# liuhatry/xflow

Measured on AMD Instinct MI355X. Metric: samples/sec (whole node) + logloss, LR-FTRL Criteo-1TB shape at 1/2/4/8 MI355X, higher is better.
Workload: dtype fp32; 1 GPU; model=LR-FTRL, global_batch=262144, seq_len=39, parallelism=dp1+table-shard1, rows_per_gpu=262144, nnz_per_row=39, slices=1, grad_layout=unique_lr, hashed_features=1000000000, table_slots_per_gpu=2147483648, backend=hip:gfx950:0, a2a_transport=none, input_overlap=False, table_growths=0

## Files before the change

### csrc/engine/engine.cpp

```cpp
#include <cstdlib>
#include "xflow/engine.h"

#include <algorithm>
#include <atomic>
#include <chrono>
#include <cmath>
#include <cstdio>
#include <cstring>
#include <thread>
#include <fstream>
#include <stdexcept>

namespace xflow {

namespace {

uint64_t next_pow2(uint64_t v) {
  uint64_t p = 1;
  while (p < v) p <<= 1;
  return p;
}

constexpr char kMagic[8] = {'X', 'F', 'L', 'O', 'W', 'T', 'B', '1'};

// ... 43 lines not shown
  table_.split = 0;
  table_.cap = 1ull << log2_cap_;
  const u64 seg = 1ull << table_.seg_log2;
  table_.probe_limit = seg < kMaxProbe ? seg : kMaxProbe;
  max_segs_ = cfg_.table_grow ? (1ull << max_log2_cap_) >> table_.seg_log2 : table_.cap >> table_.seg_log2;
  table_bytes_ = (size_t)table_.cap * table_.L.stride * sizeof(u32);
  table_.words = static_cast<u32*>(
      be.table_reserve((size_t)(max_segs_ << table_.seg_log2) * table_.L.stride * sizeof(u32),
                       max_segs_ > (table_.cap >> table_.seg_log2)));
  table_range_.e = this;
  table_.words = static_cast<u32*>(be.table_commit(table_.words, table_bytes_));
  overflow_ = mon_.alloc_zero(be, 4) + 2;
  table_.size = reinterpret_cast<unsigned long long*>(mon_.get());
  table_.overflow = overflow_ + 1;
  be.table_clear(table_);
  if (cfg_.admit_min_count > 1) {
    const int top = cfg_.table_grow ? max_log2_cap_ : log2_cap_;
    admit_.log2 = cfg_.admit_log2 ? cfg_.admit_log2 : (top + 1 < kAdmitMaxLog2 ? top + 1 : kAdmitMaxLog2);
    if (admit_.log2 < kAdmitBlockLog2) admit_.log2 = kAdmitBlockLog2;
    admit_.min_count = cfg_.admit_min_count;
    admit_.counters = admit_counters_.alloc_zero(be, (size_t)1 << admit_.log2);
  }
  std::memset(snaps_.alloc(be, kSnaps), 0, sizeof(HostSnap) * kSnaps);

  const int64_t nnz = cfg_.max_nnz;
  scratch_.cap = next_pow2((uint64_t)((double)nnz * cfg_.scratch_factor) + 1);
  scratch_.keys = scratch_keys_.alloc(be, scratch_.cap);
  be.fill_u64(scratch_.keys, kEmptyKey, scratch_.cap);
  scratch_.stamps = scratch_stamps_.alloc_zero(be, scratch_.cap);
  scratch_.claims = scratch_claims_.alloc_zero(be, 1);
  scratch_.rebuild_at = scratch_.cap / 2;
  scratch_.epoch = 0;
  if (be.is_gpu()) {
    scratch_.ctl = scratch_ctl_.alloc(be, 5);
    unsigned long long c0[5] = {scratch_.cap, 0ull, 0ull, 0ull, 0ull};
    be.copy_h2d(scratch_.ctl, c0, sizeof(c0));
  }
  block_counts_.alloc(be, scratch_.cap / 4096 + 1);

  const int ps = cfg_.model.pstride();
  uniq_keys_.alloc(be, nnz);
  uniq_slot_.alloc(be, nnz);
  use_worker_set(0);
  const uint64_t rows1 = scratch_.cap + 1;
  grad_.alloc_zero(be, rows1 * slice_cap_ * ps);
  tmask_.alloc_zero(be, rows1);
  const bool fm_ref = cfg_.model.kind == kFM && cfg_.model.fm_math == kFmReference;
  const bool fm_std = cfg_.model.kind == kFM && cfg_.model.fm_math == kFmStandard;
  const bool mvm = cfg_.model.kind == kMVM && cfg_.model.kernel_dim() >= 2;
  if (be.is_gpu() && (cfg_.model.kind == kLR || fm_ref || fm_std || mvm)) {
    const bool vec = fm_std || mvm;
    const int kd = cfg_.model.kernel_dim();
    const int nv = fm_ref ? 2 : (fm_std ? 1 + kd : (mvm ? kd : 1));
    const int shift = red_shift(nv);
    const int recw = vec ? vec_rec_words(nv) / 2 : nv;
    const int group_rows = fm_ref ? kFmGroupRows : (vec ? kFmStdMinGroupRows : kLrGroupRows);
    const uint64_t dests = scratch_.cap * (uint64_t)slice_cap_;
    const int vd = nv - 1;
    const int maxb = vec && (cfg_.max_rows + fmstd_block(vd) - 1) / fmstd_block(vd) <= kSegMaxGroups
                         ? vec_red_max_buckets(vd)
                         : kRedMaxBuckets;
    red_maxb_ = vec ? maxb : 0;
    int nb = (int)((dests + (1ull << shift) - 1) >> shift);
    int nsub = 1;
    while ((uint64_t)nb > (uint64_t)maxb * nsub) nsub <<= 1;
    if (nsub > 1) nb = maxb;
    red_nsub_ = nsub;
    if (nb <= maxb && dests < (1ull << 32)) {
      const int64_t groups = (cfg_.max_rows + group_rows - 1) / group_rows;
// ... 1205 lines not shown
    be_->copy_d2h(&c0, admit_.counters + p.c0, 1);
    be_->copy_d2h(&c1, admit_.counters + p.c1, 1);
    out[i] = c0 < c1 ? c0 : c1;
  }
  return out;
}

void Engine::admit_export(uint8_t* dst) {
  if (admit_.counters) be_->copy_d2h(dst, admit_.counters, admit_bytes());
}

void Engine::admit_import(const uint8_t* src) {
  if (!admit_.counters) throw std::runtime_error("admit_import: admission is off");
  be_->synchronize();
  be_->copy_h2d(admit_.counters, src, admit_bytes());
  be_->synchronize();
}

std::vector<u32> Engine::server_slots(int buf) {
  if (buf < 0 || buf >= kSrvBufs) throw std::invalid_argument("server buffer must be in [0, kSrvBufs)");
  const SrvBuf& sb = srv_[buf];
  std::vector<u32> out((size_t)(sb.n > 0 ? sb.n : 0));
  if (!out.empty()) be_->copy_d2h(out.data(), sb.slots, sizeof(u32) * out.size());
  return out;
}

int64_t Engine::scratch_capacity() {
  if (!scratch_.ctl) return (int64_t)scratch_.cap;
  unsigned long long c = 0;
  be_->copy_d2h(&c, scratch_.ctl, sizeof(c));
  return (int64_t)c;
}

bool Engine::overflowed() {
  u32 o[2] = {0, 0};
  be_->copy_d2h(o, overflow_, sizeof(o));
  return o[0] || o[1];
}

BatchView Engine::synth_batch(const SynthArgs& a0, int64_t slice_rows) {
  SynthArgs a = a0;
  if (a.rows > cfg_.max_rows || a.rows * a.fields > cfg_.max_nnz)
    throw std::invalid_argument("synth batch exceeds engine capacity");
  if (a.col_stride > 0 && (a.col_stride < a.rows || (!a0.keys && a.col_stride != a.rows)))
    throw std::invalid_argument("synth: col_stride must be >= rows (== rows for staging)");
  a.keys = a0.keys ? a0.keys : st_keys_;
  a.labels = a0.labels ? a0.labels : st_labels_;
  if (!a0.fgid) a.fgid = cfg_.model.kind == kMVM ? st_fgid_.get() : nullptr;
  be_->synth_batch(a);
  BatchView b;
  b.keys = a.keys;
  b.labels = a.labels;
  b.fgid = a.fgid;
  b.rows = a.rows;
  b.nnz = a.rows * a.fields;
  b.nnz_per_row = a.fields;
  b.slice_rows = slice_rows;
  b.col_stride = a.col_stride;
  return b;
}

BatchView Engine::stage_host_batch(const BatchView& h) {
  if (h.rows > cfg_.max_rows || h.nnz > cfg_.max_nnz)
    throw std::invalid_argument("host batch exceeds engine capacity");
  BatchView b = h;
  be_->copy_h2d(st_keys_, h.keys, sizeof(u64) * h.nnz);
// ... 228 lines not shown
```

### csrc/hip/kernels_table.hip

```cpp
#include <cstdlib>
#include <cstring>
#include <type_traits>

#include "kernels.h"
#include "hip_util.h"

namespace xflow {
namespace hip {

constexpr u32 kNoSlot = 0xFFFFFFFFu;
constexpr int kGroupGridCap = 8192;

__device__ __forceinline__ u64 active_cap(const ScratchView& sv) {
  return sv.ctl ? (u64)sv.ctl[0] : sv.cap;
}

__device__ __forceinline__ u64 batch_cap(const ScratchView& sv) {
  return sv.ctl ? (u64)sv.ctl[3] : sv.cap;
}

__device__ __forceinline__ bool batch_spilled(const ScratchView& sv) {
  return sv.ctl && sv.ctl[4] == (unsigned long long)sv.epoch;
}

// ... 158 lines not shown
    else pos[i] = (u32)e;
  }
  block_count_add<kBlock>(sv.claims, claimed);
}

constexpr int kCompactItems = 16;
constexpr int kCompactChunk = kBlock * kCompactItems;
constexpr int kScanBlock = 1024;

__device__ __forceinline__ unsigned int compact_hits(const ScratchView& sv, u64 base, u64 cap,
                                                     unsigned int& cnt) {
  unsigned int hit = 0;
  cnt = 0;
  if (base >= cap) return 0;
  const uint4 q = *reinterpret_cast<const uint4*>(sv.stamps + base);
  const u32 w[4] = {q.x, q.y, q.z, q.w};
  const u32 e = sv.epoch & 0xFFu;
#pragma unroll
  for (int j = 0; j < 16; ++j) hit |= (unsigned int)(((w[j >> 2] >> (8 * (j & 3))) & 0xFFu) == e) << j;
  cnt = __popc(hit);
  return hit;
}

__global__ void __launch_bounds__(kBlock) k_compact_count(ScratchView sv,
                                                          unsigned int* __restrict__ counts) {
  const u64 base = (u64)blockIdx.x * kCompactChunk + (u64)threadIdx.x * kCompactItems;
  unsigned int cnt;
  compact_hits(sv, base, batch_spilled(sv) ? sv.cap : active_cap(sv), cnt);
  unsigned int tot;
  block_exclusive_scan<kBlock>(cnt, &tot);
  if (threadIdx.x == 0) counts[blockIdx.x] = tot;
}

__global__ void __launch_bounds__(kScanBlock) k_compact_scan(
    unsigned int* __restrict__ counts, int nb, unsigned long long* __restrict__ n_out,
    unsigned long long* __restrict__ claims, unsigned long long* __restrict__ ctl,
    u64 cap_alloc, unsigned long long* __restrict__ n_copy,
    unsigned long long* __restrict__ cap_out, u32 epoch) {
  if (ctl) {
    const u64 lim = ctl[4] == epoch ? cap_alloc : (u64)ctl[0];
    const u64 nbl = (lim + kCompactChunk - 1) / kCompactChunk;
    if (nbl < (u64)nb) nb = (int)nbl;
  }
  unsigned long long carry = 0;
  for (int c0 = 0; c0 < nb; c0 += kScanBlock) {
    int i = c0 + (int)threadIdx.x;
    unsigned int v = i < nb ? counts[i] : 0u;
    unsigned int tot;
    unsigned int ex = block_exclusive_scan<kScanBlock>(v, &tot);
    if (i < nb) counts[i] = (unsigned int)(carry + ex);
    carry += tot;
  }
  if (threadIdx.x == 0) {
    *n_out = carry;
    if (n_copy) *n_copy = carry;
    if (ctl) {
      const u64 mx = ctl[1] > carry ? ctl[1] : carry;
      ctl[1] = mx;
      u64 want = kScratchMinCap;
      while (want < kScratchHeadroom * mx && want < cap_alloc) want <<= 1;
      if (want > cap_alloc) want = cap_alloc;
      const u64 cur = ctl[0];
      const bool rebuild = *claims > cur / 2 || want > cur || want * 4 <= cur;
      ctl[3] = cur;
      ctl[2] = rebuild ? want : 0ull;
      if (rebuild) {
        ctl[0] = want;
        *claims = 0ull;
      }
    }
    if (cap_out) *cap_out = ctl && ctl[4] != epoch ? ctl[3] : cap_alloc;
  }
}

__global__ void __launch_bounds__(kBlock) k_compact_write(ScratchView sv,
                                                          const unsigned int* __restrict__ offs,
                                                          u64* __restrict__ uk,
                                                          u32* __restrict__ up,
                                                          u32* __restrict__ inv) {
  const u64 base = (u64)blockIdx.x * kCompactChunk + (u64)threadIdx.x * kCompactItems;
  unsigned int cnt;
  unsigned int hit = compact_hits(sv, base, batch_spilled(sv) ? sv.cap : batch_cap(sv), cnt);
  unsigned int tot;
  unsigned int ex = block_exclusive_scan<kBlock>(cnt, &tot);
  unsigned long long dst = (unsigned long long)offs[blockIdx.x] + ex;
  u32 iv[kCompactItems];
  u64 kv[kCompactItems];
  if (hit) {
    const ulonglong2* kp = reinterpret_cast<const ulonglong2*>(sv.keys + base);
#pragma unroll
    for (int q = 0; q < kCompactItems / 2; ++q) {
      const ulonglong2 v = kp[q];
      kv[2 * q] = v.x;
      kv[2 * q + 1] = v.y;
    }
  }
#pragma unroll
  for (int j = 0; j < kCompactItems; ++j) {
    iv[j] = 0xFFFFFFFFu;
    if (!(hit & (1u << j))) continue;
    u64 s = base + (u64)j;
    uk[dst] = kv[j];
    up[dst] = (u32)s;
    iv[j] = (u32)dst;
    ++dst;
  }
  if (inv && hit) {
    uint4* ip = reinterpret_cast<uint4*>(inv + base);
#pragma unroll
    for (int j = 0; j < kCompactItems / 4; ++j)
      ip[j] = make_uint4(iv[4 * j], iv[4 * j + 1], iv[4 * j + 2], iv[4 * j + 3]);
  }
  const u64 fresh = sv.ctl ? (u64)sv.ctl[2] : 0ull;
  if (base < fresh) {
    ulonglong2* kp = reinterpret_cast<ulonglong2*>(sv.keys + base);
#pragma unroll
    for (int j = 0; j < kCompactItems / 2; ++j) kp[j] = make_ulonglong2(kEmptyKey, kEmptyKey);
  }
}

constexpr int kRemapPer = 4;

__global__ void __launch_bounds__(kBlock) k_remap_pos(u32* __restrict__ pos, int64_t nnz,
                                                      const u32* __restrict__ inv, u32 none) {
  const int64_t i = ((int64_t)blockIdx.x * kBlock + threadIdx.x) * kRemapPer;
  auto map = [&](u32 u) { return u == 0xFFFFFFFFu ? none : u; };
  if (i + kRemapPer <= nnz) {
    uint4 p[kRemapPer / 4];
#pragma unroll
    for (int q = 0; q < kRemapPer / 4; ++q) p[q] = reinterpret_cast<const uint4*>(pos + i)[q];
    u32 u[kRemapPer];
#pragma unroll
    for (int q = 0; q < kRemapPer / 4; ++q) {
      u[4 * q] = inv[p[q].x];
      u[4 * q + 1] = inv[p[q].y];
      u[4 * q + 2] = inv[p[q].z];
      u[4 * q + 3] = inv[p[q].w];
    }
#pragma unroll
    for (int q = 0; q < kRemapPer / 4; ++q)
      reinterpret_cast<uint4*>(pos + i)[q] =
          make_uint4(map(u[4 * q]), map(u[4 * q + 1]), map(u[4 * q + 2]), map(u[4 * q + 3]));
  } else {
    for (int64_t j = i; j < nnz; ++j) pos[j] = map(inv[pos[j]]);
  }
}

void launch_remap_pos(u32* pos, int64_t nnz, const u32* inv, u32 none, hipStream_t st) {
  if (nnz <= 0) return;
  if (reinterpret_cast<uintptr_t>(pos) & 15) throw std::runtime_error("remap_pos: pos must be 16-byte aligned");
// ... 35 lines not shown

void launch_partition_counts(const ScratchView& s, const u32* chunk_offsets,
                             const int64_t* n_uniq, int64_t* counts, int64_t seq, hipStream_t st) {
  if (s.parts < 2 || s.parts > kMaxParts) throw std::runtime_error("partition_counts: bad parts");
  hipLaunchKernelGGL(k_partition_counts, dim3(1), dim3(kPartBlock), 0, st, s, chunk_offsets,
                     n_uniq, counts, seq);
  XF_HIP_CHECK(hipGetLastError());
}

void launch_dedup(const u64* keys, int64_t nnz, ScratchView s, DedupOut o, hipStream_t st) {
  if (nnz <= 0) return;
  if (!s.ctl || s.grow > 0.0f) {
    if (s.ctl) hipLaunchKernelGGL(k_scratch_grow, dim3(1), dim3(1), 0, st, s.ctl, s.cap, s.grow);
    hipLaunchKernelGGL(k_scratch_maybe_clear, dim3(grid_for((int64_t)s.cap)), dim3(kBlock), 0, st,
                       s.keys, s.cap, s.claims, s.rebuild_at, s.ctl);
    hipLaunchKernelGGL(k_scratch_claims_reset, dim3(1), dim3(1), 0, st, s.claims, s.rebuild_at,
                       s.ctl);
  }
  int g1 = (int)((nnz + kDedupChunk - 1) / kDedupChunk);
  if (o.lead) {
    if (nnz % kDedupChunk || s.cap >= kLeadBit || s.parts != 1)
      throw std::runtime_error("dedup: the leader handoff needs whole tiles and < 2^31 slots");
    hipLaunchKernelGGL(k_dedup_insert<true>, dim3(g1), dim3(kBlock), 0, st, keys, nnz, s, o.pos,
                       o.overflow);
  } else {
    hipLaunchKernelGGL(k_dedup_insert<false>, dim3(g1), dim3(kBlock), 0, st, keys, nnz, s, o.pos,
                       o.overflow);
  }
  if (!o.block_counts) throw std::runtime_error("dedup: block_counts workspace missing");
  int g2 = (int)((s.cap + kCompactChunk - 1) / kCompactChunk);
  hipLaunchKernelGGL(k_compact_count, dim3(g2), dim3(kBlock), 0, st, s, o.block_counts);
  hipLaunchKernelGGL(k_compact_scan, dim3(1), dim3(kScanBlock), 0, st, o.block_counts, g2,
                     reinterpret_cast<unsigned long long*>(o.n_uniq), s.claims, s.ctl, s.cap,
                     reinterpret_cast<unsigned long long*>(o.n_uniq_copy), o.cap_out, s.epoch);
  hipLaunchKernelGGL(k_compact_write, dim3(g2), dim3(kBlock), 0, st, s, o.block_counts,
                     o.uniq_keys, o.uniq_pos, o.inv);
  XF_HIP_CHECK(hipGetLastError());
}

__global__ void k_fill_u64(u64* p, u64 v, size_t n) {
  const size_t stride = (size_t)gridDim.x * blockDim.x;
  for (size_t i = (size_t)blockIdx.x * blockDim.x + threadIdx.x; i < n; i += stride) p[i] = v;
}

struct SmallBytes {
  unsigned char b[256];
};

__global__ void k_upload_small(unsigned char* __restrict__ dst, SmallBytes v, int n) {
  for (int i = threadIdx.x; i < n; i += blockDim.x) dst[i] = v.b[i];
}

void launch_upload_small(void* dst, const void* src, size_t bytes, hipStream_t st) {
  if (bytes == 0) return;
  if (bytes > sizeof(SmallBytes)) throw std::runtime_error("upload_small: at most 256 bytes");
  SmallBytes v;
  std::memcpy(v.b, src, bytes);
  hipLaunchKernelGGL(k_upload_small, dim3(1), dim3(64), 0, st, static_cast<unsigned char*>(dst),
                     v, (int)bytes);
  XF_HIP_CHECK(hipGetLastError());
}

__global__ void k_download_small(unsigned char* __restrict__ dst,
                                 const unsigned char* __restrict__ src, int n) {
  for (int i = threadIdx.x; i < n; i += blockDim.x) dst[i] = src[i];
}

// ... 1740 lines not shown
```

### csrc/include/xflow/backend.h

```cpp
#pragma once

#include <stddef.h>
#include <stdint.h>

#include <memory>
#include <stdexcept>
#include <string>
#include <vector>

#include "xflow/types.h"

namespace xflow {

constexpr u64 kMaxProbe = 1ull << 16;
constexpr int kMaxSegLog2 = 20;

struct TableView {
  u32* words = nullptr;
  u64 cap = 0;
  TableLayout L;
  unsigned long long* size = nullptr;
  u32* overflow = nullptr;
  u64 probe_limit = 0;
  int seg_log2 = 0;
  int level = 0;
  u64 split = 0;
};

XF_HD u64 table_home(const TableView& t, u64 h) {
  const u64 hi = h >> t.seg_log2;
  u64 b = hi & ((1ull << t.level) - 1);
  if (b < t.split) b = hi & ((2ull << t.level) - 1);
  return (b << t.seg_log2) | (h & ((1ull << t.seg_log2) - 1));
}
XF_HD u64 table_next(const TableView& t, u64 s) {
  const u64 m = (1ull << t.seg_log2) - 1;
  return (s & ~m) | ((s + 1) & m);
}

struct ScratchView {
  u64* keys = nullptr;
  unsigned char* stamps = nullptr;
  u64 cap = 0;
  u32 epoch = 1;
  unsigned long long* claims = nullptr;
  u64 rebuild_at = 0;
  unsigned long long* ctl = nullptr;
  float grow = 0.0f;
  int parts = 1;
  int home_bits = 0;
};
constexpr int kMaxParts = 1024;

constexpr int kCountBits = 40;
constexpr int64_t kSeqMask = (1ll << 23) - 1;
XF_HD int64_t encode_count(int64_t count, int64_t seq) {
  return ((seq & kSeqMask) << kCountBits) | (count + 1);
}
constexpr u32 kStampEpochs = 255;
constexpr u64 kScratchHeadroom = 4;
constexpr u64 kScratchMinCap = 1ull << 16;

struct DedupOut {
  u32* pos = nullptr;
  u64* uniq_keys = nullptr;
  u32* uniq_pos = nullptr;
  int64_t* n_uniq = nullptr;
  u32* overflow = nullptr;
  u32* block_counts = nullptr;
  u32* inv = nullptr;
  int64_t* n_uniq_copy = nullptr;
  unsigned long long* cap_out = nullptr;
  bool lead = false;
};
constexpr int kLeadTile = 1024;
constexpr u32 kLeadBit = 0x80000000u;
constexpr int kLeadMaxFields = 40;

struct CsrOut {
  u32* off = nullptr;
  u32* cnt = nullptr;
  void* ent = nullptr;
  int slog2 = 0;
  const int32_t* rows = nullptr;
  int ew = 0, P = 0;
};
constexpr int csr_row_words(int P) { return (1 + P + 3) & ~3; }

struct MvmDup {
  float* rec = nullptr;
  u32* n = nullptr;
  u32* vmax = nullptr;
  long long* acc = nullptr;
  u32* claim = nullptr;
// ... 416 lines not shown
```

### csrc/include/xflow/engine.h

```cpp
#pragma once

#include <memory>
#include <string>
#include <vector>

#include "xflow/backend.h"
#include "xflow/device_buffer.h"

namespace xflow {

struct EngineConfig {
  ModelSpec model;
  OptSpec opt;
  int table_log2_cap = 20;
  int64_t max_rows = 1 << 16;
  int64_t max_nnz = 1 << 22;
  int max_slices = 1;
  bool sum_slices = false;
  double scratch_factor = 2.5;
  int device = -1;
  bool table_grow = true;
  double grow_load = 0.8;
  double grow_start = 0.6;
  int max_log2_cap = 0;
  int monitor_lag = 2;
  int owner_group = 0;
  bool csr = true;
  int admit_min_count = 1;
  int admit_log2 = 0;
  bool lead_handoff = true;
};

struct StepInputs {
  bool gpu = false;
  bool remaps = false;
  bool red_pairs = false;
  bool red_rowv = false;
  bool fm_vals = false;
  bool csr = true;
  bool sum_slices = false;
  int kind = kLR;
  int fm_math = kFmReference;
  TableLayout L;
  double scratch_cap = 0.0, max_nnz = 0.0, max_rows = 0.0;
  int pstride = 1, slice_cap = 1;
  int kdim = 1;
  bool lead_handoff = true;
  bool field_major = false;
  double rows = 0.0, fields = 0.0;
};

enum class GradPath : int { kCsr = 0, kUniqueLR, kUniqueFmBC, kUniqueRows, kSlotSums, kSlotRows };
const char* grad_path_name(GradPath g);

struct StepPlan {
  int S = 1, groups = 1, Sf = 1;
  int csr_slog2 = -1;
  bool csr_rows = false;
  GradPath grad = GradPath::kSlotRows;
  bool masks = false;
  bool upos = false;
  bool lr16 = false;
  bool lr16s = false;
// ... 52 lines not shown
  int csr_entry_bytes() const {
    return csr_full_rows() ? 4 * csr_row_words(table_.L.P) : (fm_vals_ ? 12 : 8);
  }
  bool csr_full_rows() const {
    return (cfg_.model.kind == kFM && cfg_.model.fm_math == kFmStandard) ||
           (cfg_.model.kind == kMVM && cfg_.model.kernel_dim() >= 2);
  }
  void w_forward_backward_csr(const BatchView& b, const float* pulled, int64_t n_send,
                              int S_global, int wb, bool pack, u32* cnt_out, void* ent_out,
                              const int64_t* counts, int world, bool encoded, int64_t* totals_out);
  void s_apply_csr(const u64* recv_keys, const u32* recv_cnt, const void* recv_ent,
                   const std::vector<int64_t>& src_offsets, int S, int buf = 0);
  void s_apply(const u64* recv_keys, const float* recv_grads, const u32* recv_masks,
               const std::vector<int64_t>& src_offsets, int S, int buf = 0);
  void w_finish();

  EvalMetrics eval_metrics(const float* pctr, const float* labels, int64_t n) {
    return be_->eval_metrics(pctr, labels, n);
  }
  GroupedEval eval_grouped(const float* pctr, const float* labels, const u64* groups, int64_t n,
                           GroupTable* table = nullptr) {
    return be_->eval_grouped(pctr, labels, groups, n, table);
  }
  void row_group_keys(const BatchView& b, int field, u64* out) {
    if (!b.fgid && b.row_ptr)
      throw std::invalid_argument("row_group_keys: a CSR batch needs its field ids (fgid)");
    be_->row_group_keys(b, field, out);
  }

  LossStats read_stats(bool reset, int which = 0);
  int64_t n_unique();
  int64_t table_size();
  int64_t scratch_capacity();
  uint64_t table_capacity() const { return table_.cap; }
  size_t table_bytes() const { return table_bytes_; }
  bool overflowed();
  int64_t table_growths() const { return growths_; }
  int64_t csr_steps() const { return csr_steps_; }
  void csr_debug(std::vector<u32>& off, std::vector<u32>& cnt, std::vector<u32>& words);
  int64_t table_splits() const { return splits_; }
  size_t admit_bytes() const { return admit_.counters ? (size_t)1 << admit_.log2 : 0; }
  int admit_log2() const { return admit_.counters ? admit_.log2 : 0; }
  std::vector<uint8_t> admit_counts(const std::vector<u64>& keys);
  void admit_export(uint8_t* dst);
  void admit_import(const uint8_t* src);
  std::vector<u32> server_slots(int buf);
  std::vector<int64_t> table_geometry() const {
    return {table_.seg_log2, table_.level, (int64_t)table_.split,
            (int64_t)(table_.cap >> table_.seg_log2)};
  }
  size_t table_committed() const;
  double grow_seconds() const { return grow_s_; }
  int64_t monitor_waits() const { return monitor_waits_; }
  double monitor_wait_seconds() const { return monitor_wait_s_; }
  void count_records(bool on);
  int64_t take_records();
  void grow_table(int log2_cap);
  int64_t prune(float max_n = -1.0f);
  int64_t pruned_keys() const { return pruned_keys_; }
  void end_step();
  int64_t nonzero_weights() { return be_->table_nonzero(table_, cfg_.opt); }
  int pstride() const { return cfg_.model.pstride(); }
  int value_width() const { return vstride_; }
  int grad_width() const { return sharded_fm_compact() ? 2 : pstride(); }
  int slices_of(const BatchView& b) const;
  static constexpr int kSliceGroup = 32;
// ... 218 lines not shown
```

### csrc/python/module.cpp

```cpp
#include <pybind11/numpy.h>
#include <pybind11/pybind11.h>
#include <pybind11/stl.h>

#include <algorithm>
#include <atomic>
#include <charconv>
#include <cstdint>
#include <cstdio>
#include <cstring>
#include <thread>
#include <vector>
#include <string>

#include "../comm/async_ps.h"
#include "../comm/rccl_comm.h"
#include "../comm/sharded_step.h"
#include "xflow/engine.h"
#include "xflow/reader.h"
#include "xflow/trainer.h"

namespace py = pybind11;
using namespace xflow;

namespace {
// ... 325 lines not shown
               std::string s = h;
               v.emplace_back(s.begin(), s.end());
             }
             a.connect(v);
           })
      .def("start", &AsyncPS::start)
      .def("train_step", &AsyncPS::train_step, py::call_guard<py::gil_scoped_release>())
      .def("eval_step",
           [](AsyncPS& a, const BatchView& b, uintptr_t pctr) { return a.eval_step(b, P<float>(pctr)); },
           py::call_guard<py::gil_scoped_release>())
      .def("finish", &AsyncPS::finish, py::call_guard<py::gil_scoped_release>())
      .def("stop", &AsyncPS::stop, py::call_guard<py::gil_scoped_release>())
      .def("log", [](const AsyncPS& a) { return to_np(a.log()); })
      .def_property_readonly("serving", &AsyncPS::serving)
      .def_property_readonly("transport", &AsyncPS::transport)
      .def_property_readonly("csr", &AsyncPS::csr)
      .def_readonly("steps", &AsyncPS::steps)
      .def_readonly("evals", &AsyncPS::evals)
      .def_readwrite("bytes_moved", &AsyncPS::bytes_moved)
      .def_readwrite("max_staleness", &AsyncPS::max_staleness)
      .def_readwrite("max_lead", &AsyncPS::max_lead)
      .def_readwrite("wait_slot_s", &AsyncPS::wait_slot_s)
      .def_readwrite("wait_pull_s", &AsyncPS::wait_pull_s)
      .def_readwrite("sync_s", &AsyncPS::sync_s)
      .def_readonly("served_pulls", &AsyncPS::served_pulls)
      .def_readonly("applied_pushes", &AsyncPS::applied_pushes)
      .def_readonly("server_busy_s", &AsyncPS::server_busy_s);

  py::class_<Engine>(m, "Engine")
      .def(py::init([](py::dict model, py::dict opt, int table_log2_cap, int64_t max_rows,
                       int64_t max_nnz, int max_slices, bool sum_slices, double scratch_factor,
                       int device, bool table_grow, double grow_load, int max_log2_cap,
                       int monitor_lag, int owner_group, double grow_start, bool csr,
                       int admit_min_count, int admit_log2, bool lead_handoff) {
             EngineConfig c;
             c.lead_handoff = lead_handoff;
             c.admit_min_count = admit_min_count;
             c.admit_log2 = admit_log2;
             c.owner_group = owner_group;
             c.csr = csr;
             c.table_grow = table_grow;
             c.grow_load = grow_load;
             c.grow_start = grow_start;
             c.max_log2_cap = max_log2_cap;
             c.monitor_lag = monitor_lag;
             c.model = model_from(model);
             c.opt = opt_from(opt);
             c.table_log2_cap = table_log2_cap;
             c.max_rows = max_rows;
             c.max_nnz = max_nnz;
             c.max_slices = max_slices;
             c.sum_slices = sum_slices;
             c.scratch_factor = scratch_factor;
             c.device = device;
             return new Engine(c);
           }),
           py::arg("model"), py::arg("opt"), py::arg("table_log2_cap") = 20,
           py::arg("max_rows") = 1 << 16, py::arg("max_nnz") = 1 << 22,
           py::arg("max_slices") = 1, py::arg("sum_slices") = false,
           py::arg("scratch_factor") = 2.5, py::arg("device") = -1,
           py::arg("table_grow") = true, py::arg("grow_load") = 0.8, py::arg("max_log2_cap") = 0,
           py::arg("monitor_lag") = 2, py::arg("owner_group") = 0, py::arg("grow_start") = 0.6,
           py::arg("csr") = true, py::arg("admit_min_count") = 1, py::arg("admit_log2") = 0,
           py::arg("lead_handoff") = true)
      .def_property_readonly("admit_bytes", &Engine::admit_bytes)
      .def_property_readonly("admit_log2", &Engine::admit_log2)
      .def("admit_counts",
           [](Engine& e, py::array_t<uint64_t, py::array::c_style | py::array::forcecast> keys) {
             std::vector<u64> k(keys.data(), keys.data() + keys.size());
             return to_np(e.admit_counts(k));
           })
      .def("admit_export",
           [](Engine& e) {
             py::array_t<uint8_t> a((py::ssize_t)e.admit_bytes());
             uint8_t* p = a.mutable_data();
             {
               py::gil_scoped_release nogil;
               e.admit_export(p);
             }
             return a;
           })
      .def("admit_import",
           [](Engine& e, py::array_t<uint8_t, py::array::c_style | py::array::forcecast> a) {
             if ((size_t)a.size() != e.admit_bytes())
               throw std::invalid_argument("admit_import: size mismatch");
             const uint8_t* p = a.data();
             py::gil_scoped_release nogil;
             e.admit_import(p);
           })
      .def("server_slots", [](Engine& e, int buf) { return to_np(e.server_slots(buf)); },
           py::arg("buf") = 0)
      .def_property_readonly("table_growths", &Engine::table_growths)
      .def_property_readonly("csr_steps", &Engine::csr_steps)
      .def("step_plan",
           [](const Engine& e, int S, int64_t rows, int64_t fields, bool field_major) {
             return plan_dict(e.plan(S, rows, fields, field_major));
           },
// ... 197 lines not shown
             for (size_t f = 0; f < F; ++f) {
               a.width[f] = width[f];
               a.col_off[f] = col_off[f];
               a.dict[f] = P<const u64>(dict[f]);
               a.fgid_col[f] = fgid_col[f];
             }
             a.keys = P<u64>(keys);
             a.labels = P<float>(labels);
             a.fgid = P<int32_t>(fgid);
             e.backend().unpack_block(a);
           },
           py::arg("block"), py::arg("rows"), py::arg("width"), py::arg("col_off"),
           py::arg("dict"), py::arg("fgid_col"), py::arg("keys"), py::arg("labels"),
           py::arg("fgid") = 0, py::call_guard<py::gil_scoped_release>())
      .def("field_major",
           [](Engine& e, uintptr_t src, uintptr_t dst, int64_t rows, int F, int elem_bytes,
              bool widen) {
             e.backend().field_major(P<const void>(src), P<void>(dst), rows, F, elem_bytes, widen);
           },
           py::arg("src"), py::arg("dst"), py::arg("rows"), py::arg("F"), py::arg("elem_bytes"),
           py::arg("widen") = false, py::call_guard<py::gil_scoped_release>())
      .def("read_stats",
           [](Engine& e, bool reset, int which) { return stats_dict(e.read_stats(reset, which)); },
           py::arg("reset") = false, py::arg("which") = 0)
      .def("csr_debug",
           [](Engine& e) {
             std::vector<u32> o, c, w;
             e.csr_debug(o, c, w);
             return py::make_tuple(to_np(o), to_np(c), to_np(w));
           })
      .def("n_unique", &Engine::n_unique)
      .def("table_size", &Engine::table_size)
      .def("scratch_capacity", &Engine::scratch_capacity)
      .def("overflowed", &Engine::overflowed)
      .def("nonzero_weights", &Engine::nonzero_weights)
      .def("export_table",
           [](Engine& e) {
             const int64_t n = e.table_size();
             py::array_t<uint64_t> k((py::ssize_t)n);
             py::array_t<uint32_t> w((py::ssize_t)(n * e.state_words()));
             u64* kp = reinterpret_cast<u64*>(k.mutable_data());
             u32* wp = reinterpret_cast<u32*>(w.mutable_data());
             {
               py::gil_scoped_release nogil;
               e.export_into(kp, wp, n);
             }
             return py::make_tuple(k, w);
           })
      .def("import_table",
           [](Engine& e, py::array_t<uint64_t, py::array::c_style | py::array::forcecast> keys,
              py::array_t<uint32_t, py::array::c_style | py::array::forcecast> words) {
             const int64_t n = (int64_t)keys.size();
             if ((int64_t)words.size() != n * e.state_words())
               throw std::invalid_argument("import_table: size mismatch");
             const u64* kp = reinterpret_cast<const u64*>(keys.data());
             const u32* wp = reinterpret_cast<const u32*>(words.data());
             py::gil_scoped_release nogil;
             e.import_from(kp, wp, n);
           })
      .def("save", &Engine::save, py::call_guard<py::gil_scoped_release>())
      .def("load", &Engine::load, py::call_guard<py::gil_scoped_release>())
      .def("synth_batch",
           [](Engine& e, int64_t rows, std::vector<uint64_t> vocab, std::vector<float> zipf,
              uint64_t hash_space, uint64_t seed, uint64_t step, float scale, float bias,
              int64_t slice_rows, uintptr_t keys, uintptr_t labels, uintptr_t fgid,
              bool field_major) {
// ... 137 lines not shown
```

### xflow_amd/config.py

```python
from __future__ import annotations

import dataclasses
import os
from dataclasses import dataclass, field

MODEL_KINDS = {"lr": 0, "fm": 1, "mvm": 2}
MODEL_NAMES = {v: k for k, v in MODEL_KINDS.items()}
OPT_KINDS = {"ftrl": 0, "sgd": 1}
FM_MATH = {"reference": 0, "standard": 1}
MVM_MATH = {"compat": 0, "fixed": 1}


def model_kind(m) -> int:
    if isinstance(m, int):
        if m not in MODEL_NAMES:
            raise ValueError(f"model index must be 0 (LR), 1 (FM) or 2 (MVM), got {m}")
        return m
    m = str(m).lower()
    if m in ("0", "1", "2"):
        return int(m)
    if m not in MODEL_KINDS:
        raise ValueError(f"unknown model {m!r}; expected lr/fm/mvm")
    return MODEL_KINDS[m]

# ... 23 lines not shown
    alpha: float = 5e-2
    beta: float = 1.0
    lambda1: float = 5e-5
    lambda2: float = 10.0
    lr: float = 1e-3
    sgd_v_init: float = 1e-3
    v_init_scale: float = 1e-2
    seed: int = 0x5EED

    def native(self) -> dict:
        d = dataclasses.asdict(self)
        d["kind"] = OPT_KINDS[self.kind]
        return d


@dataclass
class EngineConfig:
    table_log2_cap: int = 22
    max_rows: int = 1 << 16
    max_nnz: int = 1 << 22
    max_slices: int = 1
    sum_slices: bool = False
    scratch_factor: float = 2.5
    table_grow: bool = True
    grow_load: float = 0.8
    grow_start: float = 0.6
    max_log2_cap: int = 0
    monitor_lag: int = 2
    owner_group: int = 0
    csr: bool = True
    admit_min_count: int = 1
    admit_log2: int = 0
    lead_handoff: bool = True


@dataclass
class TrainConfig:
    train_prefix: str = ""
    test_prefix: str = ""
    epochs: int = 60
    threads: int = 0
    train_block_bytes: int = 2 << 20
    block_rows: int = 0
    fixed_width: bool = True
    resident: bool = False
    copy_threads: int = 8
    gpu_parse: bool = False
    test_block_bytes: int = 0
    serial_slices: bool = False
    keep_remainder: bool = False
    mvm_predict_compat: bool = False
    init_push: bool = True
    pred_dir: str = "."
    write_pred: bool = True
    checkpoint_dir: str = ""
    save_every: int = 0
    resume_dir: str = ""
    prune_every: int = 0
    prune_max_n: float = -1.0
    gauc_field: int = -1
    metrics_file: str = ""
    async_p2p: bool = False
    async_ps: bool = False
    staleness: int = 1
    model: ModelConfig = field(default_factory=ModelConfig)
    optim: OptimConfig = field(default_factory=OptimConfig)
# ... 13 lines not shown
```

### xflow_amd/engine.py

```python
from __future__ import annotations

from dataclasses import dataclass
from typing import Optional

import numpy as np
import torch

from xflow_amd import native
from xflow_amd.config import EngineConfig, ModelConfig, OptimConfig


@dataclass
class Batch:

    keys: torch.Tensor
    labels: torch.Tensor
    row_ptr: Optional[torch.Tensor] = None
    fgid: Optional[torch.Tensor] = None
    nnz_per_row: int = 0
    slice_rows: int = 0
    field_major: bool = False

    @property
    def rows(self) -> int:
# ... 72 lines not shown


def _device_index(device: torch.device) -> int:
    if device.type == "cpu":
        return -1
    if device.type != "cuda":
        raise ValueError(f"unsupported device {device}")
    return device.index if device.index is not None else torch.cuda.current_device()


class Engine:

    def __init__(self, model: ModelConfig | None = None, optim: OptimConfig | None = None,
                 engine: EngineConfig | None = None, device: str | torch.device = "cpu"):
        self.model = model or ModelConfig()
        self.optim = optim or OptimConfig()
        self.cfg = engine or EngineConfig()
        self.device = torch.device(device)
        if self.device.type == "cuda":
            native.require_hip()
            if self.device.index is None:
                self.device = torch.device("cuda", torch.cuda.current_device())
        n = native.load()
        self._e = n.Engine(self.model.native(), self.optim.native(),
                           table_log2_cap=self.cfg.table_log2_cap, max_rows=self.cfg.max_rows,
                           max_nnz=self.cfg.max_nnz, max_slices=self.cfg.max_slices,
                           sum_slices=self.cfg.sum_slices, scratch_factor=self.cfg.scratch_factor,
                           device=_device_index(self.device), table_grow=self.cfg.table_grow,
                           grow_load=self.cfg.grow_load, max_log2_cap=self.cfg.max_log2_cap,
                           monitor_lag=self.cfg.monitor_lag, owner_group=self.cfg.owner_group,
                           grow_start=self.cfg.grow_start, csr=self.cfg.csr,
                           admit_min_count=self.cfg.admit_min_count,
                           admit_log2=self.cfg.admit_log2,
                           lead_handoff=self.cfg.lead_handoff)
        if self.is_gpu != (self.device.type == "cuda"):
            raise RuntimeError("native engine backend does not match the requested device")

    @property
    def native(self):
        return self._e

    @property
    def is_gpu(self) -> bool:
        return bool(self._e.is_gpu)

    @property
    def backend_name(self) -> str:
        return self._e.backend_name

    @property
    def pstride(self) -> int:
        return int(self._e.pstride)

    @property
    def grad_width(self) -> int:
        return int(self._e.grad_width)

    @property
    def value_width(self) -> int:
        return int(self._e.value_width)

    @property
    def params_per_key(self) -> int:
        return int(self._e.P)

    def _sync_stream(self) -> None:
        if self.is_gpu:
# ... 203 lines not shown

    def take_records(self) -> int:
        self._sync_stream()
        return int(self._e.take_records())

    @property
    def monitor_wait_seconds(self) -> float:
        return float(self._e.monitor_wait_seconds)

    def grow_table(self, log2_cap: int) -> None:
        self._sync_stream()
        self._e.grow_table(int(log2_cap))

    def prune(self, max_n: float | None = None) -> int:
        self._sync_stream()
        return int(self._e.prune(-1.0 if max_n is None else float(max_n)))

    @property
    def pruned_keys(self) -> int:
        return int(self._e.pruned_keys)

    def end_step(self) -> None:
        self._sync_stream()
        self._e.end_step()

    def n_unique(self) -> int:
        self._sync_stream()
        return int(self._e.n_unique())

    def scratch_capacity(self) -> int:
        self._sync_stream()
        return int(self._e.scratch_capacity())

    def overflowed(self) -> bool:
        self._sync_stream()
        return bool(self._e.overflowed())

    def nonzero_weights(self) -> int:
        self._sync_stream()
        return int(self._e.nonzero_weights())

    def download_small(self, dst: torch.Tensor, src: torch.Tensor) -> None:
        if self.is_gpu and not dst.is_pinned():
            raise ValueError("download_small: dst must be pinned host memory")
        if dst.numel() * dst.element_size() < src.numel() * src.element_size():
            raise ValueError("download_small: dst too small")
        self._sync_stream()
        self._e.download_small(dst.data_ptr(), src.contiguous().data_ptr(),
                               src.numel() * src.element_size())

    def eval_metrics(self, pctr: torch.Tensor, labels: torch.Tensor) -> dict:
        if pctr.device != self.device or labels.device != self.device:
            raise ValueError("eval_metrics: tensors must be on the engine's device")
        p = pctr.contiguous().float()
        y = labels.contiguous().float()
        if p.numel() != y.numel():
            raise ValueError("eval_metrics: pctr and labels differ in length")
        self._sync_stream()
        return dict(self._e.eval_metrics(p.data_ptr(), y.data_ptr(), int(p.numel())))

    def eval_grouped(self, pctr: torch.Tensor, labels: torch.Tensor, groups: torch.Tensor,
                     per_group: bool = False) -> dict:
        if pctr.device != self.device or labels.device != self.device or \
                groups.device != self.device:
            raise ValueError("eval_grouped: tensors must be on the engine's device")
        if groups.dtype != torch.int64:
# ... 50 lines not shown
```

Measured before the change: 633.8 million samples/s.

## Carry current batch keys across scratch dedup-table rebuilds

When the GPU scratch hash table used for per-batch key dedup hits its claim threshold without needing a resize, the rebuild now rewrites the keys seen in the current batch instead of clearing every slot. Claims restart at the carried count, and the rebuild threshold drops to three eighths of capacity when carry is on. The aim is to cut the cost of reinserting hot keys after every clear and to make full rebuilds less frequent. In exchange the table holds more stale entries, so probe chains may get longer. Two control words and a stats accessor are added, and the feature is on by default.

```diff
diff --git a/csrc/engine/engine.cpp b/csrc/engine/engine.cpp
--- a/csrc/engine/engine.cpp
+++ b/csrc/engine/engine.cpp
@@ -99,9 +99,11 @@
   scratch_.rebuild_at = scratch_.cap / 2;
   scratch_.epoch = 0;
   if (be.is_gpu()) {
-    scratch_.ctl = scratch_ctl_.alloc(be, 5);
-    unsigned long long c0[5] = {scratch_.cap, 0ull, 0ull, 0ull, 0ull};
+    scratch_.ctl = scratch_ctl_.alloc(be, kScratchCtlWords);
+    unsigned long long c0[kScratchCtlWords] = {scratch_.cap};
+    static_assert(kScratchCtlWords >= 8, "ScratchView::ctl[0..7]");
     be.copy_h2d(scratch_.ctl, c0, sizeof(c0));
+    scratch_.carry = cfg_.scratch_carry;
   }
   block_counts_.alloc(be, scratch_.cap / 4096 + 1);
 
@@ -1373,6 +1375,22 @@
   return (int64_t)c;
 }
 
+ScratchStats Engine::scratch_stats() {
+  ScratchStats s;
+  unsigned long long claims = 0;
+  be_->copy_d2h(&claims, scratch_.claims, sizeof(claims));
+  s.occupancy = (int64_t)claims;
+  s.capacity = (int64_t)scratch_.cap;
+  if (scratch_.ctl) {
+    unsigned long long c[kScratchCtlWords];
+    be_->copy_d2h(c, scratch_.ctl, sizeof(c));
+    s.capacity = (int64_t)c[0];
+    s.rebuilds = (int64_t)c[6];
+    s.carried = (int64_t)c[7];
+  }
+  return s;
+}
+
 bool Engine::overflowed() {
   u32 o[2] = {0, 0};
   be_->copy_d2h(o, overflow_, sizeof(o));
diff --git a/csrc/hip/kernels_table.hip b/csrc/hip/kernels_table.hip
--- a/csrc/hip/kernels_table.hip
+++ b/csrc/hip/kernels_table.hip
@@ -214,11 +214,14 @@
   if (threadIdx.x == 0) counts[blockIdx.x] = tot;
 }
 
+constexpr u64 kCarryRebuildEighths = 3;
+static_assert(kCarryRebuildEighths <= 4, "stale claims <= cur / 2 at a batch start");
+
 __global__ void __launch_bounds__(kScanBlock) k_compact_scan(
     unsigned int* __restrict__ counts, int nb, unsigned long long* __restrict__ n_out,
     unsigned long long* __restrict__ claims, unsigned long long* __restrict__ ctl,
     u64 cap_alloc, unsigned long long* __restrict__ n_copy,
-    unsigned long long* __restrict__ cap_out, u32 epoch) {
+    unsigned long long* __restrict__ cap_out, u32 epoch, bool carry_on) {
   if (ctl) {
     const u64 lim = ctl[4] == epoch ? cap_alloc : (u64)ctl[0];
     const u64 nbl = (lim + kCompactChunk - 1) / kCompactChunk;
@@ -243,12 +246,19 @@
       while (want < kScratchHeadroom * mx && want < cap_alloc) want <<= 1;
       if (want > cap_alloc) want = cap_alloc;
       const u64 cur = ctl[0];
-      const bool rebuild = *claims > cur / 2 || want > cur || want * 4 <= cur;
+      const bool resize = want > cur || want * 4 <= cur;
+      const u64 full_at = carry_on ? cur * kCarryRebuildEighths / 8 : cur / 2;
+      const bool rebuild = *claims > full_at || resize;
+      const bool keep = carry_on && rebuild && !resize && ctl[4] != epoch &&
+                        carry * kScratchHeadroom <= cur;
       ctl[3] = cur;
       ctl[2] = rebuild ? want : 0ull;
+      ctl[5] = keep ? 1ull : 0ull;
       if (rebuild) {
         ctl[0] = want;
-        *claims = 0ull;
+        *claims = keep ? carry : 0ull;
+        ctl[6] += 1ull;
+        ctl[7] = keep ? carry : 0ull;
       }
     }
     if (cap_out) *cap_out = ctl && ctl[4] != epoch ? ctl[3] : cap_alloc;
@@ -296,8 +306,15 @@
   const u64 fresh = sv.ctl ? (u64)sv.ctl[2] : 0ull;
   if (base < fresh) {
     ulonglong2* kp = reinterpret_cast<ulonglong2*>(sv.keys + base);
-#pragma unroll
-    for (int j = 0; j < kCompactItems / 2; ++j) kp[j] = make_ulonglong2(kEmptyKey, kEmptyKey);
+    if (hit && sv.ctl[5]) {
+#pragma unroll
+      for (int j = 0; j < kCompactItems / 2; ++j)
+        kp[j] = make_ulonglong2(hit & (1u << (2 * j)) ? kv[2 * j] : kEmptyKey,
+                                hit & (1u << (2 * j + 1)) ? kv[2 * j + 1] : kEmptyKey);
+    } else {
+#pragma unroll
+      for (int j = 0; j < kCompactItems / 2; ++j) kp[j] = make_ulonglong2(kEmptyKey, kEmptyKey);
+    }
   }
 }
 
@@ -399,7 +416,8 @@
   hipLaunchKernelGGL(k_compact_count, dim3(g2), dim3(kBlock), 0, st, s, o.block_counts);
   hipLaunchKernelGGL(k_compact_scan, dim3(1), dim3(kScanBlock), 0, st, o.block_counts, g2,
                      reinterpret_cast<unsigned long long*>(o.n_uniq), s.claims, s.ctl, s.cap,
-                     reinterpret_cast<unsigned long long*>(o.n_uniq_copy), o.cap_out, s.epoch);
+                     reinterpret_cast<unsigned long long*>(o.n_uniq_copy), o.cap_out, s.epoch,
+                     s.carry);
   hipLaunchKernelGGL(k_compact_write, dim3(g2), dim3(kBlock), 0, st, s, o.block_counts,
                      o.uniq_keys, o.uniq_pos, o.inv);
   XF_HIP_CHECK(hipGetLastError());
diff --git a/csrc/include/xflow/backend.h b/csrc/include/xflow/backend.h
--- a/csrc/include/xflow/backend.h
+++ b/csrc/include/xflow/backend.h
@@ -46,6 +46,7 @@
   unsigned long long* claims = nullptr;
   u64 rebuild_at = 0;
   unsigned long long* ctl = nullptr;
+  bool carry = false;
   float grow = 0.0f;
   int parts = 1;
   int home_bits = 0;
@@ -60,6 +61,7 @@
 constexpr u32 kStampEpochs = 255;
 constexpr u64 kScratchHeadroom = 4;
 constexpr u64 kScratchMinCap = 1ull << 16;
+constexpr int kScratchCtlWords = 8;
 
 struct DedupOut {
   u32* pos = nullptr;
diff --git a/csrc/include/xflow/engine.h b/csrc/include/xflow/engine.h
--- a/csrc/include/xflow/engine.h
+++ b/csrc/include/xflow/engine.h
@@ -29,6 +29,14 @@
   int admit_min_count = 1;
   int admit_log2 = 0;
   bool lead_handoff = true;
+  bool scratch_carry = true;
+};
+
+struct ScratchStats {
+  int64_t capacity = 0;
+  int64_t occupancy = 0;
+  int64_t rebuilds = 0;
+  int64_t carried = 0;
 };
 
 struct StepInputs {
@@ -147,6 +155,7 @@
   int64_t n_unique();
   int64_t table_size();
   int64_t scratch_capacity();
+  ScratchStats scratch_stats();
   uint64_t table_capacity() const { return table_.cap; }
   size_t table_bytes() const { return table_bytes_; }
   bool overflowed();
diff --git a/csrc/python/module.cpp b/csrc/python/module.cpp
--- a/csrc/python/module.cpp
+++ b/csrc/python/module.cpp
@@ -381,9 +381,11 @@
                        int64_t max_nnz, int max_slices, bool sum_slices, double scratch_factor,
                        int device, bool table_grow, double grow_load, int max_log2_cap,
                        int monitor_lag, int owner_group, double grow_start, bool csr,
-                       int admit_min_count, int admit_log2, bool lead_handoff) {
+                       int admit_min_count, int admit_log2, bool lead_handoff,
+                       bool scratch_carry) {
              EngineConfig c;
              c.lead_handoff = lead_handoff;
+             c.scratch_carry = scratch_carry;
              c.admit_min_count = admit_min_count;
              c.admit_log2 = admit_log2;
              c.owner_group = owner_group;
@@ -411,7 +413,7 @@
            py::arg("table_grow") = true, py::arg("grow_load") = 0.8, py::arg("max_log2_cap") = 0,
            py::arg("monitor_lag") = 2, py::arg("owner_group") = 0, py::arg("grow_start") = 0.6,
            py::arg("csr") = true, py::arg("admit_min_count") = 1, py::arg("admit_log2") = 0,
-           py::arg("lead_handoff") = true)
+           py::arg("lead_handoff") = true, py::arg("scratch_carry") = true)
       .def_property_readonly("admit_bytes", &Engine::admit_bytes)
       .def_property_readonly("admit_log2", &Engine::admit_log2)
       .def("admit_counts",
@@ -675,6 +677,16 @@
       .def("n_unique", &Engine::n_unique)
       .def("table_size", &Engine::table_size)
       .def("scratch_capacity", &Engine::scratch_capacity)
+      .def("scratch_stats",
+           [](Engine& e) {
+             const ScratchStats s = e.scratch_stats();
+             py::dict d;
+             d["capacity"] = s.capacity;
+             d["occupancy"] = s.occupancy;
+             d["rebuilds"] = s.rebuilds;
+             d["carried"] = s.carried;
+             return d;
+           })
       .def("overflowed", &Engine::overflowed)
       .def("nonzero_weights", &Engine::nonzero_weights)
       .def("export_table",
diff --git a/xflow_amd/config.py b/xflow_amd/config.py
--- a/xflow_amd/config.py
+++ b/xflow_amd/config.py
@@ -79,6 +79,7 @@
     admit_min_count: int = 1
     admit_log2: int = 0
     lead_handoff: bool = True
+    scratch_carry: bool = True
 
 
 @dataclass
diff --git a/xflow_amd/engine.py b/xflow_amd/engine.py
--- a/xflow_amd/engine.py
+++ b/xflow_amd/engine.py
@@ -128,7 +128,8 @@
                            grow_start=self.cfg.grow_start, csr=self.cfg.csr,
                            admit_min_count=self.cfg.admit_min_count,
                            admit_log2=self.cfg.admit_log2,
-                           lead_handoff=self.cfg.lead_handoff)
+                           lead_handoff=self.cfg.lead_handoff,
+                           scratch_carry=self.cfg.scratch_carry)
         if self.is_gpu != (self.device.type == "cuda"):
             raise RuntimeError("native engine backend does not match the requested device")
 
@@ -398,6 +399,10 @@
         self._sync_stream()
         return int(self._e.scratch_capacity())
 
+    def scratch_stats(self) -> dict:
+        self._sync_stream()
+        return {k: int(v) for k, v in self._e.scratch_stats().items()}
+
     def overflowed(self) -> bool:
         self._sync_stream()
         return bool(self._e.overflowed())
```

New measurement: 669.3 million samples/s (median of 6 runs). 5.6% higher.
